# ElesionKyrie/Extreme-Video-Compression-With-Prediction-Using-Pre-trainded-Diffusion-Models-

Hardware: AMD Instinct MI355X
Metric: decoded frames/sec (128x128x30) at q3 (higher is better)
Workload: dtype f32

## Files before the change

### extreme-video-compression-with-prediction-using-pre-trainded-diffusion-models-_amd/csrc/api.hip

```cpp
#include <hip/hip_runtime.h>
#include <string.h>
#include "../../include/evc_hip.h"

extern "C" const char* evc_version(void) { return "evc-hip 0.1"; }
extern "C" const char* evc_arch(void) { return "gfx950"; }

extern "C" int evc_device_ok(void) {
    int dev = 0;
    if (hipGetDevice(&dev) != hipSuccess) return 0;
    hipDeviceProp_t prop;
    if (hipGetDeviceProperties(&prop, dev) != hipSuccess) return 0;
    return strncmp(prop.gcnArchName, "gfx950", 6) == 0 ? 1 : 0;
}

__global__ void clock_probe_kernel(unsigned long long* out, unsigned long long ref_ticks, const unsigned* stop) {
    const unsigned long long r0 = wall_clock64(), c0 = clock64();
    unsigned long long r1 = r0;
    while (r1 - r0 < ref_ticks) {
        __builtin_amdgcn_s_sleep(64);
        r1 = wall_clock64();
        if (stop && __hip_atomic_load(stop, __ATOMIC_RELAXED, __HIP_MEMORY_SCOPE_AGENT) != 0u) break;
    }
    const unsigned long long c1 = clock64();
    if (threadIdx.x == 0) { out[0] = c1 - c0; out[1] = r1 - r0; }
}

extern "C" int evc_clock_probe(unsigned long long* out2, int spin_us, const unsigned* stop, void* stream) {
    if (!out2 || spin_us <= 0 || spin_us > 10000000) return EVC_EINVAL;
    hipLaunchKernelGGL(clock_probe_kernel, dim3(1), dim3(64), 0, (hipStream_t)stream, out2, (unsigned long long)spin_us * 100ull, stop);
    return hipGetLastError() == hipSuccess ? EVC_OK : EVC_ELAUNCH;
}
```

### extreme-video-compression-with-prediction-using-pre-trainded-diffusion-models-_amd/csrc/conv_igemm.hip

```cpp
#include <hip/hip_runtime.h>
#include <stdint.h>
#include <stdio.h>
#include "../../include/evc_hip.h"

typedef float f32x16 __attribute__((ext_vector_type(16)));
typedef __attribute__((address_space(3))) void lds_void;
typedef const __attribute__((address_space(1))) void glb_void;

#ifndef EVC_CONV_TAIL
#define EVC_CONV_TAIL 1
#endif
#ifndef EVC_CONV_TM1
#define EVC_CONV_TM1 1
#endif
#ifndef EVC_SPLIT_WIDE_TILES
#define EVC_SPLIT_WIDE_TILES 1
#endif

#ifndef EVC_SPLIT_INTERLEAVE
#define EVC_SPLIT_INTERLEAVE 5
#endif

namespace {

// ... 1128 lines not shown
        }
    }
}

__device__ __forceinline__ void wide_epilogue(const ConvK& p, f32x16 (&acc)[4][3], char* lds, int m0, int n0, int split,
                                              int wave, int lane, bool tail) {
    const bool partial = p.splits > 1 || tail;
    if (partial) wide_epilogue_t<true, false, false, false>(p, acc, lds, m0, n0, split, wave, lane, tail);
    else if (p.act_out != EVC_ACT_NONE) wide_epilogue_t<false, true, true, true>(p, acc, lds, m0, n0, split, wave, lane, tail);
    else if (p.res && p.stats) wide_epilogue_t<false, true, true, false>(p, acc, lds, m0, n0, split, wave, lane, tail);
    else if (p.stats) wide_epilogue_t<false, false, true, false>(p, acc, lds, m0, n0, split, wave, lane, tail);
    else if (p.res) wide_epilogue_t<false, true, false, false>(p, acc, lds, m0, n0, split, wave, lane, tail);
    else wide_epilogue_t<false, false, false, false>(p, acc, lds, m0, n0, split, wave, lane, tail);
}

#ifndef EVC_WIDE_VMEM_EVERY
#define EVC_WIDE_VMEM_EVERY 36
#endif
#ifndef EVC_WIDE_BDIST
#define EVC_WIDE_BDIST 1
#endif
#ifndef EVC_WIDE_BUFFER_LOADS
#define EVC_WIDE_BUFFER_LOADS 0
#endif
#ifndef EVC_WIDE_ABL
#define EVC_WIDE_ABL 0
#endif
#ifdef EVC_WIDE_STAMPS
__device__ unsigned long long g_wide_stamps[8192 * 8];
#define EVC_STAMP(k) if (threadIdx.x == 0) g_wide_stamps[(blockIdx.x & 8191) * 8 + (k)] = __builtin_readcyclecounter();
#else
#define EVC_STAMP(k)
#endif
template <int MODE, int NU, bool X2>
__global__ __launch_bounds__(256, 1) void conv_wide_kernel(ConvK p) {
    typedef Split<2> SP;
    typedef f16x8 vec;
    constexpr int TM = 4, TN = 3, BM = 256, BN = 192, RB = 32;
    constexpr bool HAS_COEF = MODE == MODE_AFFINE || MODE == MODE_AFFINE_SILU;
    extern __shared__ __attribute__((aligned(16))) char smem_b[];
    const int W = p.W, SW = W + 2;
    const int R = BM / W;
    const int SPX = (R + 2) * SW;
    const int APL = SPX * RB;
    const int HPL = SPX * 16;
    char* const As = smem_b;

    const int tid = threadIdx.x;
    const int lane = tid & 63;
    const int wave = __builtin_amdgcn_readfirstlane(tid >> 6);
    const int wm = wave >> 1, wn = wave & 1;
    const int l31 = lane & 31, half = lane >> 5;

#ifdef EVC_WIDE_STAGGER_TEST
    if (blockIdx.x < 256) for (int q = 0; q < (int)((blockIdx.x >> 3) & 3) * EVC_WIDE_STAGGER_TEST; ++q) __builtin_amdgcn_s_sleep(127);
#endif
    EVC_STAMP(0)
    const bool tail = (int)blockIdx.x >= p.tail_first;
    const int tq = tail ? ((int)blockIdx.x - p.tail_first) / p.tail_splits : 0;
    const int m0 = (tail ? p.tail_first + tq : (int)blockIdx.x) * BM;
    const int n0 = blockIdx.y * BN;
    const int split = tail ? (int)blockIdx.x - p.tail_first - tq * p.tail_splits : (int)blockIdx.z;
    const int sps = tail ? p.tail_sps : p.steps_per_split;
    const int c_begin = p.cut_chunk ? (split ? p.cut_chunk : 0) : min(p.nchunk, split * (sps / 9));
    const int c_end = p.cut_chunk ? (split ? p.nchunk : p.cut_chunk) : min(p.nchunk, c_begin + sps / 9);

    const int bimg = m0 / p.HW;
    const int y0 = (m0 - bimg * p.HW) / W;
// ... 73 lines not shown
            cs[0] = *reinterpret_cast<const float4*>(p.coef_s + co);
            cs[1] = *reinterpret_cast<const float4*>(p.coef_s + co + 4);
        }
    };
    auto stage_store = [&](int k, int buf) {
        vec pl[2];
        SP::split(transform<MODE>(xr[k][0], ca[0], cs[0], sval[k]), transform<MODE>(xr[k][1], ca[1], cs[1], sval[k]), xscale, pl);
        char* A = As + buf * 2 * APL + slds[k];
        *reinterpret_cast<vec*>(A) = pl[0];
        *reinterpret_cast<vec*>(A + APL) = pl[1];
    };
    auto read_a = [&](int i, const char* img, int toff) {
        a[i][0] = *reinterpret_cast<const vec*>(img + abase[i] + toff);
        a[i][1] = *reinterpret_cast<const vec*>(img + APL + abase[i] + toff);
    };

    f32x16 acc[TM][TN];
#pragma unroll
    for (int i = 0; i < TM; ++i)
#pragma unroll
        for (int j = 0; j < TN; ++j)
#pragma unroll
            for (int r = 0; r < 16; ++r) acc[i][j][r] = 0.f;

    vec b[3][TN][2];
    const bool early = !X2 && c_begin < c_end;
    if (early) {
        coef_load(c_begin);
#pragma unroll
        for (int k = 0; k < NU; ++k) stage_load(k, c_begin);
        load_b(b[0], c_begin, 0);
    }
    EVC_STAMP(5)
    {
        const int nimg = X2 ? 3 : 2;
        const int per_img = (R + 2) * 2 * 4;
        for (int u = tid; u < nimg * per_img; u += 256) {
            const int img = u / per_img, q = u - img * per_img;
            const int ph = q & 3, side = (q >> 2) & 1, row = q >> 3;
            const int spx = row * SW + (side ? W + 1 : 0);
            *reinterpret_cast<float4*>(As + img * 2 * APL + (ph >> 1) * APL + (ph & 1) * HPL + spx * 16) = make_float4(0.f, 0.f, 0.f, 0.f);
        }
    }
    __syncthreads();

#define EVC_PIN(x) asm volatile("" : "+v"(x))
#define EVC_PIN4(f) asm volatile("" : "+v"((f).x), "+v"((f).y), "+v"((f).z), "+v"((f).w))
#define EVC_WIDE_MFMA_I(I, BB)                                                                          \
    _Pragma("unroll") for (int t_ = 0; t_ < SP::NTERM; ++t_)                                            \
        _Pragma("unroll") for (int j = 0; j < TN; ++j)                                                  \
            acc[I][j] = SP::mfma(a[I][SP::qa(t_)], BB[j][SP::qb(t_)], acc[I][j]);

    if constexpr (X2) {
        const int nch2 = (p.x2_C0 + p.x2_C1) / KC;
        const int nsp = tail ? p.tail_splits : p.splits;
        const int per = (nch2 + nsp - 1) / nsp;
        const int c2b = min(nch2, split * per), c2e = min(nch2, c2b + per);
        float s2 = 1.0f;
        {
            const float bb = sqrtf(__uint_as_float(p.x2_bound[bound_index(p, m0)]));
            if (!(bb < 3.0e38f)) s2 = __builtin_nanf("");
            else if (bb > 0.f) s2 = ldexpf(1.0f, 6 - ilogbf(bb));
        }
        const float xscale2 = F16_ACT_SCALE * s2;
        const unsigned slab2 = 2u * planeB;
        float4 x2r[2][2][2];
        unsigned x2o0[2], x2o1[2];
        int x2l[2];
#pragma unroll
        for (int k = 0; k < 2; ++k) {
            const int pp = (tid + 256 * k) >> 1;
            const int r = pp / W, x = pp - r * W;
            x2o0[k] = ((unsigned)(m0 + pp) * (unsigned)p.x2_ld0 + 8u * kh) * 4u;
            x2o1[k] = ((unsigned)(m0 + pp) * (unsigned)p.x2_ld1 + 8u * kh) * 4u;
            x2l[k] = kh * HPL + ((r + 1) * SW + x + 1) * 16;
        }
        auto load2 = [&](int c, float4 (&xr2)[2][2]) {
            const int cc = c * KC;
            const bool first = cc < p.x2_C0;
            const char* src = reinterpret_cast<const char*>(first ? p.x2_src0 : p.x2_src1);
            const unsigned cb = (unsigned)(first ? cc : cc - p.x2_C0) * 4u;
#pragma unroll
            for (int k = 0; k < 2; ++k) {
                const unsigned o = (first ? x2o0[k] : x2o1[k]) + cb;
                xr2[k][0] = *reinterpret_cast<const float4*>(src + o);
                xr2[k][1] = *reinterpret_cast<const float4*>(src + o + 16);
            }
        };
        auto store2 = [&](int buf, float4 (&xr2)[2][2]) {
            const float4 z = make_float4(0.f, 0.f, 0.f, 0.f);
#pragma unroll
            for (int k = 0; k < 2; ++k) {
                vec pl[2];
                SP::split(transform<MODE_PLAIN>(xr2[k][0], z, z, true), transform<MODE_PLAIN>(xr2[k][1], z, z, true), xscale2, pl);
                char* A = As + buf * 2 * APL + x2l[k];
                *reinterpret_cast<vec*>(A) = pl[0];
                *reinterpret_cast<vec*>(A + APL) = pl[1];
            }
        };
        vec b2[2][TN][2];
        auto load_b2 = [&](vec (&bb)[TN][2], int c) {
            const char* wt = p.x2_w + (unsigned)c * slab2;
#pragma unroll
            for (int j = 0; j < TN; ++j) {
                bb[j][0] = *reinterpret_cast<const vec*>(wt + wlane + j * 32 * RB);
                bb[j][1] = *reinterpret_cast<const vec*>(wt + planeB + wlane + j * 32 * RB);
            }
        };
        const int n2 = c2e - c2b;
        if (n2 > 0) {
            const auto clampc = [&](int c) { return min(c, c2e - 1); };
            load2(c2b, x2r[0]);
            load2(clampc(c2b + 1), x2r[1]);
            load_b2(b2[0], c2b);
            store2(0, x2r[0]);
            store2(1, x2r[1]);
            load2(clampc(c2b + 2), x2r[0]);
            load2(clampc(c2b + 3), x2r[1]);
            __syncthreads();
#pragma unroll
            for (int i = 0; i < TM; ++i) read_a(i, As, tap_off(4));
            int ring = 0;
#define EVC_WIDE_X2_STEP(BCUR, BNXT, XR)                                                                    \
            {                                                                                           \
                const int rn1 = ring == 2 ? 0 : ring + 1, rn2 = rn1 == 2 ? 0 : rn1 + 1;                 \
                _Pragma("unroll") for (int j = 0; j < TN; ++j) { EVC_PIN(BCUR[j][0]); EVC_PIN(BCUR[j][1]); } \
                _Pragma("unroll") for (int k = 0; k < 2; ++k) { EVC_PIN4(XR[k][0]); EVC_PIN4(XR[k][1]); } \
                load_b2(BNXT, clampc(c + 1));                                                           \
                const char* An = As + rn1 * 2 * APL;                                                    \
                _Pragma("unroll") for (int i = 0; i < TM; ++i) {                                        \
                    EVC_PIN(a[i][0]); EVC_PIN(a[i][1]);                                                 \
                    EVC_WIDE_MFMA_I(i, BCUR)                                                            \
                    read_a(i, An, tap_off(4));                                                          \
                }                                                                                       \
                store2(rn2, XR);                                                       \
                _Pragma("unroll") for (int m = 0; m < 36; ++m) {                                        \
                    if (m == 0) __builtin_amdgcn_sched_group_barrier(0x020, 6, 0);                      \
                    __builtin_amdgcn_sched_group_barrier(0x008, 1, 0);                                  \
                    __builtin_amdgcn_sched_group_barrier(0x402, 3, 0);                                  \
                    if (m % 9 == 8) __builtin_amdgcn_sched_group_barrier(0x100, 2, 0);                  \
                }                                                                                       \
                __builtin_amdgcn_sched_group_barrier(0x200, 4, 0);                                      \
                __builtin_amdgcn_sched_barrier(0);                                                      \
                load2(clampc(c + 4), XR);                                \
                asm volatile("s_waitcnt lgkmcnt(0)\n\ts_barrier" ::: "memory");                         \
                __builtin_amdgcn_sched_barrier(0);                                                      \
                ring = rn1;                                                                             \
            }
            int c = c2b;
            for (; c + 1 < c2e; c += 2) {
                EVC_WIDE_X2_STEP(b2[0], b2[1], x2r[0])
                ++c;
                EVC_WIDE_X2_STEP(b2[1], b2[0], x2r[1])
                --c;
            }
            if (c < c2e) EVC_WIDE_X2_STEP(b2[0], b2[1], x2r[0])
#undef EVC_WIDE_X2_STEP
        }
        __syncthreads();
        const float r = (p.x2_hdr[0] / s2) / (p.w_hdr[0] / in_scale(p, m0));
#pragma unroll
        for (int i = 0; i < TM; ++i)
#pragma unroll
            for (int j = 0; j < TN; ++j)
#pragma unroll
                for (int e = 0; e < 16; ++e) acc[i][j][e] *= r;
    }

    EVC_STAMP(6)
    if (c_begin < c_end) {
        if (!early) {
            coef_load(c_begin);
#pragma unroll
            for (int k = 0; k < NU; ++k) stage_load(k, c_begin);
            load_b(b[0], c_begin, 0);
        }
        if (EVC_WIDE_BDIST == 2) load_b(b[1], c_begin, 1);
#pragma unroll
        for (int k = 0; k < NU; ++k) stage_store(k, 0);
        EVC_STAMP(7)
        __syncthreads();
#pragma unroll
        for (int i = 0; i < TM; ++i) read_a(i, As, 0);
    }
    EVC_STAMP(1)
    for (int c = c_begin; c < c_end; ++c) {
        const int ab = (c - c_begin) & 1;
        const int cn = min(c + 1, c_end - 1);
        const char* Acur = As + ab * 2 * APL;
        const char* Anxt = As + (ab ^ 1) * 2 * APL;
#define EVC_WIDE_STEP(T, LOADK, STOREK, TAIL_CODE)                                                      \
        {                                                                                               \
// ... 30 lines not shown
        EVC_WIDE_STEP(2, 2, 0, )
        EVC_WIDE_STEP(3, 3, 1, )
        EVC_WIDE_STEP(4, -1, 2, )
        EVC_WIDE_STEP(5, -1, 3, )
        EVC_WIDE_STEP(6, -1, -1, )
        EVC_WIDE_STEP(7, -1, -1, asm volatile("s_waitcnt lgkmcnt(0)\n\ts_barrier" ::: "memory");)
        EVC_WIDE_STEP(8, -1, -1, )
#undef EVC_WIDE_STEP
    }
#undef EVC_WIDE_MFMA_I
#undef EVC_PIN
#undef EVC_PIN4

    if (EVC_WIDE_ABL & 16) {
        float sacc = 0.f;
#pragma unroll
        for (int i = 0; i < TM; ++i)
#pragma unroll
            for (int j = 0; j < TN; ++j)
#pragma unroll
                for (int e = 0; e < 16; ++e) sacc += acc[i][j][e];
        p.out[(size_t)m0 * p.ld_out + tid] = sacc;
        return;
    }
    EVC_STAMP(2)
    __syncthreads();
    wide_epilogue(p, acc, As, (EVC_WIDE_ABL & 128) ? 0 : m0, n0, split, wave, lane, tail);
#ifdef EVC_WIDE_STAMPS
    asm volatile("s_waitcnt vmcnt(0)" ::: "memory");
    EVC_STAMP(3)
    if (threadIdx.x == 0) g_wide_stamps[(blockIdx.x & 8191) * 8 + 4] = __builtin_amdgcn_s_getreg(6 | (8 << 6) | (3 << 11)) ;
#endif
}

__global__ __launch_bounds__(1024) void conv_splitk_reduce_kernel(const float* __restrict__ ws, int splits, int M,
                                                                  int Co, const float* __restrict__ bias,
                                                                  const float* __restrict__ res, int ld_res,
                                                                  float scale, int act, float* __restrict__ out,
                                                                  int ld_out, float* __restrict__ stats) {
    __shared__ float red[2][16][64];
    const int l = threadIdx.x & 63;
    const int c = blockIdx.y * 64 + l;
    const int rg = threadIdx.x >> 6;
    const int m_base = blockIdx.x * 64;
    const size_t total = (size_t)M * Co;
    float s_sum = 0.f, s_sq = 0.f;
    if (c < Co) {
        const float b = bias ? bias[c] : 0.f;
        float v[4];
        size_t idx[4];
        bool ok[4];
#pragma unroll
        for (int k = 0; k < 4; ++k) {
            const int m = m_base + rg + 16 * k;
            ok[k] = m < M;
            idx[k] = (size_t)(ok[k] ? m : 0) * Co + c;
            v[k] = 0.f;
        }
        for (int z = 0; z < splits; ++z) {
            const float* w = ws + (size_t)z * total;
#pragma unroll
            for (int k = 0; k < 4; ++k) v[k] += w[idx[k]];
        }
#pragma unroll
        for (int k = 0; k < 4; ++k) {
            if (!ok[k]) continue;
// ... 152 lines not shown
    return hipGetLastError() == hipSuccess ? EVC_OK : EVC_ELAUNCH;
}

static int conv_validate(const evc_conv_args* a) {
    if (!a || !a->src0 || !a->w_packed || !a->out) return EVC_EINVAL;
    if (a->C0 <= 0 || a->C0 % KC != 0 || a->C1 < 0 || a->C1 % KC != 0) return EVC_EINVAL;
    if (a->C1 > 0 && !a->src1) return EVC_EINVAL;
    if ((a->ld0 != 0 && (a->ld0 < a->C0 || (a->ld0 & 3))) || (a->ld1 != 0 && (a->ld1 < a->C1 || (a->ld1 & 3))))
        return EVC_EINVAL;
    if ((a->coef_a == nullptr) != (a->coef_s == nullptr)) return EVC_EINVAL;
    if (a->B <= 0 || a->H <= 0 || a->W <= 0 || a->Co <= 0) return EVC_EINVAL;
    if (a->KH <= 0 || a->KW <= 0 || !(a->KH & 1) || !(a->KW & 1)) return EVC_EINVAL;
    if (a->ld_out < a->Co || (a->res && a->ld_res < a->Co)) return EVC_EINVAL;
    if ((long long)a->B * a->H * a->W > 0x7fffffffLL) return EVC_EINVAL;
    if (a->arith != EVC_ARITH_F32 && a->arith != EVC_ARITH_BF16X6 && a->arith != EVC_ARITH_F16X3) return EVC_EINVAL;
    if (a->x2_w_packed) {
        if (!a->x2_src0 || !a->x2_bound || a->x2_C0 <= 0 || a->x2_C0 % KC != 0 || a->x2_C1 < 0 || a->x2_C1 % KC != 0) return EVC_EINVAL;
        if (a->x2_C1 > 0 && !a->x2_src1) return EVC_EINVAL;
        if ((a->x2_ld0 != 0 && (a->x2_ld0 < a->x2_C0 || (a->x2_ld0 & 3))) || (a->x2_ld1 != 0 && (a->x2_ld1 < a->x2_C1 || (a->x2_ld1 & 3))))
            return EVC_EINVAL;
    }
    return EVC_OK;
}

struct TileCfg { int tm, tn, bm, bn; long long tiles; int splits; int reuse; int wide; int steps_per_split;
                 int tail_first, tail_tiles, tail_splits, tail_sps;
                 int cut_chunk; };
static int g_wide_cut = 1;
static int g_tail_split = EVC_CONV_TAIL;
static int g_wide_tiles = EVC_SPLIT_WIDE_TILES;
static int g_no_reuse = 0;
static int g_wide_mid = 1;
static int g_wide256 = 1;
static int g_force_tm = 0;

static void split_tile_cfg(const evc_conv_args* a, long long M, long long ntile, int nsteps, TileCfg& c, bool rr_ok, bool inv) {
    const double K = (double)a->KH * a->KW * (a->C0 + a->C1);
    const bool f16 = a->arith == EVC_ARITH_F16X3 && rr_ok;
    const double E = f16 ? 20.0 : 6.0, F2 = f16 ? 1.5 : 1.0;
    const auto grid_time = [&](long long n, double sps) {
        const long long R = n / 512, rem = n - R * 512;
        return (sps + E) * ((double)R * F2 + (rem == 0 ? 0.0 : (rem <= 256 && f16 ? 1.0 : F2)));
    };
    double best = 1e300;
    int best_tm = 2, best_s = 1;
    c.tail_first = 0; c.tail_tiles = 0; c.tail_splits = 1; c.tail_sps = 0;
    for (int tm = 2; tm >= 1; --tm) {
        if (!inv && g_force_tm && tm != g_force_tm) continue;
        const long long tiles = ((M + 64 * tm - 1) / (64 * tm)) * ntile;
        const int smax = a->splits > 0 ? a->splits : (nsteps / 4 < 1 ? 1 : (nsteps / 4 > 32 ? 32 : nsteps / 4));
        for (int s = a->splits > 0 ? a->splits : 1; s <= smax; ++s) {
            const double sps = (double)((nsteps + s - 1) / s);
            const double slab_mb = (double)s * (double)M * a->Co * 4.0 / 1e6;
            const double pen = s > 1 ? 1.0 + (slab_mb > 192.0 ? 300.0 : 40.0) * s / K : 1.0;
            const double tmf = tm == 1 ? (a->KH * a->KW > 1 ? 0.5 / (rr_ok ? 0.55 : 0.75) : 0.5) : 1.0;
            const double t = grid_time(tiles * s, sps) * pen * tmf;
            if (t < best * 0.9999) { best = t; best_tm = tm; best_s = s; }
        }
    }
    c.tm = best_tm;
    c.bm = 64 * c.tm;
    c.tiles = ((M + c.bm - 1) / c.bm) * ntile;
    c.splits = best_s;
    if (!inv && rr_ok && g_tail_split && a->splits <= 0 && !g_force_tm && M % 128 == 0) {
        const long long tm_all = M / 128, wgs = tm_all * ntile;
        const long long R = wgs / 512;
        const long long main_m = R * 512 / ntile, tail_m = tm_all - main_m;
        const int unit = 3 * 9;
        if (R >= 1 && tail_m > 0 && nsteps >= 2 * unit) {
            int ts = (int)(512 / (tail_m * ntile));
            if (ts > nsteps / unit) ts = nsteps / unit;
            if (ts >= 2) {
                int sps = (nsteps + ts - 1) / ts;
                sps = (sps + 2) / 3 * 3;
                ts = (nsteps + sps - 1) / sps;
                const double t_tail = grid_time(main_m * ntile, (double)nsteps) +
                                      grid_time(tail_m * ntile * ts, (double)sps) * (1.0 + 40.0 * ts / K);
                if (ts >= 2 && t_tail < best * 0.98) {
                    c.tm = 2; c.bm = 128; c.tiles = wgs; c.splits = 1;
                    c.tail_first = (int)main_m; c.tail_tiles = (int)tail_m; c.tail_splits = ts; c.tail_sps = sps;
                }
            }
        }
    }
}

static inline bool is_split_arith(int arith) { return arith == EVC_ARITH_BF16X6 || arith == EVC_ARITH_F16X3; }
static inline int arith_planes(int arith) { return arith == EVC_ARITH_F16X3 ? 2 : 3; }
constexpr long long LDS_CAP = 160 * 1024;

static long long rr_lds_bytes(int np, int bm, int W, int bn) {
    return (long long)np * 32 * (2LL * (bm / W) * (W + 2) + 2LL * bn);
}

static long long wide_lds_bytes(int W, bool x2) { return (x2 ? 6LL : 4LL) * (256 / W + 2) * (W + 2) * 32; }

static bool wide_ok(const evc_conv_args* a, bool inv) {
    const bool mode_ok = a->coef_a ? a->act_in == EVC_ACT_SILU : a->act_in == EVC_ACT_NONE;
    return (inv || g_wide256) && mode_ok && a->arith == EVC_ARITH_F16X3 && a->KH == 3 && a->KW == 3 && a->Co % 192 == 0 &&
           (a->W == 16 || a->W == 32 || a->W == 64 || a->W == 128) && ((long long)a->H * a->W) % 256 == 0 &&
           a->ld_out % 4 == 0 && (!a->res || a->ld_res % 4 == 0);
}

static TileCfg conv_tile_cfg_at(const evc_conv_args* a, bool inv) {
    TileCfg c;
    c.wide = 0;
    c.cut_chunk = 0;
    const long long M = (long long)a->B * a->H * a->W;
    const int CoPad = evc_conv_co_pad(a->Co);
    c.tn = pick_tn(CoPad);
    c.bn = 64 * c.tn;
    const long long ntile = CoPad / c.bn;
    const int nsteps = a->KH * a->KW * ((a->C0 + a->C1) / KC);
    c.reuse = 0;
    if (is_split_arith(a->arith)) {
        const int np = arith_planes(a->arith);
        const bool rr_ok = (inv || !g_no_reuse) && a->KH == 3 && a->KW == 3 && a->W >= 4 && 128 % a->W == 0 &&
                           rr_lds_bytes(np, 128, a->W, c.bn) <= LDS_CAP;
        split_tile_cfg(a, M, ntile, nsteps, c, rr_ok, inv);
        if (rr_ok && c.tm == 2) c.reuse = 1;
        if (!inv && c.reuse && c.splits == 1 && !c.tail_tiles && g_wide_tiles && M % 256 == 0 && rr_lds_bytes(np, 256, a->W, c.bn) <= LDS_CAP) {
            const long long t256 = (M / 256) * ntile;
            if ((t256 >= 512 && t256 % 256 == 0) || t256 >= 6 * 256) {
                c.bm = 256;
                c.tiles = t256;
            }
        }
    } else {
        c.tail_first = 0; c.tail_tiles = 0; c.tail_splits = 1; c.tail_sps = 0;
        c.tm = (!EVC_CONV_TM1 || ((M + 127) / 128) * ntile >= 64) ? 2 : 1;
        if (g_force_tm && !inv) c.tm = g_force_tm;
        c.bm = 64 * c.tm;
        c.tiles = ((M + c.bm - 1) / c.bm) * ntile;
        long long splits = 1;
        if (a->splits > 0) splits = a->splits;
        else if (c.tiles < 384) {
            splits = (640 + c.tiles / 2) / c.tiles;
            const int max_by_steps = nsteps / 8 > 0 ? nsteps / 8 : 1;
            if (splits > max_by_steps) splits = max_by_steps;
            if (splits > 32) splits = 32;
            if (splits < 1) splits = 1;
        }
        c.splits = (int)splits;
    }
    if (wide_ok(a, inv) && a->splits <= 0 && (inv || !g_force_tm)) {
        const long long tm_all = M / 256, nt = a->Co / 192, wgs = tm_all * nt;
        if (wgs >= 256) {
            const int nchunk = (a->C0 + a->C1) / KC;
            c.wide = 1; c.reuse = 0; c.tm = 4; c.tn = 3; c.bm = 256; c.bn = 192; c.tiles = wgs; c.splits = 1;
            c.tail_first = 0; c.tail_tiles = 0; c.tail_splits = 1; c.tail_sps = 0;
            const long long Rr = wgs / 256;
            const long long main_m = Rr * 256 / nt, tail_m = tm_all - main_m;
            if (!inv && g_tail_split && tail_m > 0) {
                int ts = (int)(256 / (tail_m * nt));
                if (ts > nchunk / 3) ts = nchunk / 3;
                if (ts >= 2) {
                    const int cps = (nchunk + ts - 1) / ts;
                    ts = (nchunk + cps - 1) / cps;
                    c.tail_first = (int)main_m; c.tail_tiles = (int)tail_m; c.tail_splits = ts; c.tail_sps = cps * 9;
                }
            }
            c.steps_per_split = nsteps;
            return c;
        }
        if ((inv || g_wide_mid) && wgs >= 32) {
            const int nchunk = (a->C0 + a->C1) / KC;
            int best_s = 0;
            double best_t = 1e300;
            for (int sp = 1; sp <= 8 && wgs * sp <= 256 && nchunk / sp >= 4; ++sp) {
                const int cps = (nchunk + sp - 1) / sp;
                const double slab_mb = sp > 1 ? (double)sp * M * a->Co * 4.0 / 1e6 : 0.0;
                const double t = 23000.0 + 13900.0 * cps + (sp > 1 ? 2.0 * 2000.0 * (5.0 + slab_mb / 4.0) : 0.0);
                if (t < best_t) { best_t = t; best_s = sp; }
            }
            if (best_s > 0 && wgs * best_s >= 128) {
                const int cps = (nchunk + best_s - 1) / best_s;
                c.wide = 1; c.reuse = 0; c.tm = 4; c.tn = 3; c.bm = 256; c.bn = 192; c.tiles = wgs;
// ... 17 lines not shown
            }
        }
    }
    const int unit = c.reuse ? a->KW : 1;
    int sps = (nsteps + c.splits - 1) / c.splits;
    sps = (sps + unit - 1) / unit * unit;
    c.steps_per_split = sps;
    c.splits = (nsteps + sps - 1) / sps;
    return c;
}

#define EVC_INVARIANT_PLAN_REVISION 1
static TileCfg conv_tile_cfg(const evc_conv_args* a) {
    if (!a->invariant) return conv_tile_cfg_at(a, false);
    evc_conv_args r = *a;
    r.B = EVC_INVARIANT_REF_BATCH;
    TileCfg c = conv_tile_cfg_at(&r, true);
    const long long M = (long long)a->B * a->H * a->W;
    c.tiles = ((M + c.bm - 1) / c.bm) * (evc_conv_co_pad(a->Co) / c.bn);
    return c;
}

extern "C" int evc_invariant_plan_revision(void) { return EVC_INVARIANT_PLAN_REVISION; }

extern "C" int evc_conv_set_option(const char* name, int value) {
    if (!name) return EVC_EINVAL;
    const auto is = [&](const char* s) { int i = 0; while (s[i] && s[i] == name[i]) ++i; return s[i] == 0 && name[i] == 0; };
    if (is("wide_tiles")) { g_wide_tiles = value; return EVC_OK; }
    if (is("row_reuse")) { g_no_reuse = !value; return EVC_OK; }
    if (is("tail_split")) { g_tail_split = value; return EVC_OK; }
    if (is("wide256")) { g_wide256 = value; return EVC_OK; }
    if (is("wide_mid")) { g_wide_mid = value; return EVC_OK; }
    if (is("wide_cut")) { g_wide_cut = value; return EVC_OK; }
    return EVC_EINVAL;
}

extern "C" int evc_conv_fused_1x1_supported(const evc_conv_args* a) {
    if (conv_validate(a) != EVC_OK) return 0;
    if (a->arith != EVC_ARITH_F16X3 || a->KH != 3 || a->KW != 3) return 0;
    const TileCfg c = conv_tile_cfg(a);
    if (a->invariant && ((long long)a->H * a->W) % c.bm != 0) return 0;
    return (c.reuse == 1 || c.wide) ? 1 : 0;
}

extern "C" int evc_conv_kernel_name(const evc_conv_args* a, char* buf, int n) {
    if (!buf || n <= 0 || conv_validate(a) != EVC_OK) return EVC_EINVAL;
    int mode;
    if (a->coef_a) mode = a->act_in == EVC_ACT_SILU ? MODE_AFFINE_SILU : MODE_AFFINE;
    else mode = a->act_in == EVC_ACT_SILU ? MODE_SILU : a->act_in == EVC_ACT_RELU ? MODE_RELU : MODE_PLAIN;
    const TileCfg c = conv_tile_cfg(a);
    int len;
    if (c.wide) len = snprintf(buf, n, "conv_wide_kernel<%d, %d, %s>", mode, a->W == 128 ? 4 : 3, a->x2_w_packed ? "true" : "false");
    else if (is_split_arith(a->arith)) {
        const int np = arith_planes(a->arith);
        if (c.reuse) len = snprintf(buf, n, "conv_split_rr_kernel<%d, %d, %d, %d>", np, c.bm == 256 ? 4 : 2, c.tn, mode);
        else if (np == 3) len = snprintf(buf, n, "conv_split_kernel<%d, %d, %d>", c.tm, c.tn, mode);
        else len = snprintf(buf, n, "conv_splitn_kernel<2, %d, %d, %d>", c.tm, c.tn, mode);
    } else len = snprintf(buf, n, "conv_igemm_kernel<%d, %d, %d>", c.tm, c.tn, mode);
    return len;
}

extern "C" int evc_conv_choose_splits(const evc_conv_args* a) {
    if (conv_validate(a) != EVC_OK) return EVC_EINVAL;
    return conv_tile_cfg(a).splits;
}

extern "C" int evc_conv_stats_splits(const evc_conv_args* a) {
    if (conv_validate(a) != EVC_OK) return 0;
    const int HW = a->H * a->W;
    if (HW % 64 != 0) return 0;
    const TileCfg c = conv_tile_cfg(a);
    if (c.splits > 1 || c.wide) return HW / 64;
    if (a->invariant && HW % c.bm != 0) return 0;
    const long long M = (long long)a->B * HW;
    const int CoPad = evc_conv_co_pad(a->Co);
    if (M % c.bm != 0 || a->Co != CoPad || a->Co % c.bn != 0) return 0;
    return HW / (32 * c.tm);
}

extern "C" int evc_conv_plan_query(const evc_conv_args* a, evc_conv_plan* out) {
    if (!out || conv_validate(a) != EVC_OK) return EVC_EINVAL;
    const TileCfg c = conv_tile_cfg(a);
    if (evc_conv_kernel_name(a, out->kernel, (int)sizeof(out->kernel)) < 0) return EVC_EINVAL;
    out->tile_m = c.bm; out->tile_n = c.bn; out->splits = c.splits; out->steps_per_split = c.steps_per_split;
    out->cut_chunk = c.wide ? c.cut_chunk : 0;
// ... 55 lines not shown
template <int TM, int TN>
static int launch_split2(int mode, dim3 grid, size_t lds, hipStream_t st, const ConvK& k) {
#define EVC_CALL(M) hipLaunchKernelGGL((conv_splitn_kernel<2, TM, TN, M>), grid, dim3(256), lds, st, k)
    EVC_MODE_SWITCH(mode, EVC_CALL)
#undef EVC_CALL
    return EVC_OK;
}

template <int NP, int WM, int TN, int MODE>
static int launch_split_rr_one(dim3 grid, size_t lds, hipStream_t st, const ConvK& k) {
    static unsigned long long attr_done = 0;
    const int rc = ensure_dynamic_lds(reinterpret_cast<const void*>(&conv_split_rr_kernel<NP, WM, TN, MODE>), &attr_done, lds);
    if (rc != EVC_OK) return rc;
    hipLaunchKernelGGL((conv_split_rr_kernel<NP, WM, TN, MODE>), grid, dim3(128 * WM), lds, st, k);
    return EVC_OK;
}
template <int NP, int WM, int TN>
static int launch_split_rr(int mode, dim3 grid, size_t lds, hipStream_t st, const ConvK& k) {
    int rc = EVC_OK;
#define EVC_CALL(M) rc = launch_split_rr_one<NP, WM, TN, M>(grid, lds, st, k)
    EVC_MODE_SWITCH(mode, EVC_CALL)
#undef EVC_CALL
    return rc;
}

template <int MODE, int NU, bool X2>
static int launch_wide_one(dim3 grid, size_t lds, hipStream_t st, const ConvK& k) {
    static unsigned long long attr_done = 0;
    const int rc = ensure_dynamic_lds(reinterpret_cast<const void*>(&conv_wide_kernel<MODE, NU, X2>), &attr_done, lds);
    if (rc != EVC_OK) return rc;
    hipLaunchKernelGGL((conv_wide_kernel<MODE, NU, X2>), grid, dim3(256), lds, st, k);
    return EVC_OK;
}
template <int MODE>
static int launch_wide_mode(int nu, bool x2, dim3 grid, size_t lds, hipStream_t st, const ConvK& k) {
    if (nu == 4) return x2 ? launch_wide_one<MODE, 4, true>(grid, lds, st, k) : launch_wide_one<MODE, 4, false>(grid, lds, st, k);
    return x2 ? launch_wide_one<MODE, 3, true>(grid, lds, st, k) : launch_wide_one<MODE, 3, false>(grid, lds, st, k);
}
static int launch_wide(int mode, int nu, bool x2, dim3 grid, size_t lds, hipStream_t st, const ConvK& k) {
#ifdef EVC_DEV_FAST
    return launch_wide_mode<MODE_AFFINE_SILU>(nu, x2, grid, lds, st, k);
#else
    if (mode == MODE_AFFINE_SILU) return launch_wide_mode<MODE_AFFINE_SILU>(nu, x2, grid, lds, st, k);
    if (mode == MODE_PLAIN) return launch_wide_mode<MODE_PLAIN>(nu, x2, grid, lds, st, k);
    return EVC_EUNSUPPORTED;
#endif
}

#define EVC_TN_SWITCH(tn, CALL) ((tn) == 3 ? CALL(3) : (tn) == 2 ? CALL(2) : CALL(1))

static int conv2d_impl(const evc_conv_args* a, float* ws, void* stream, hipEvent_t ev_start, hipEvent_t ev_conv_end);

extern "C" int evc_conv2d_nhwc_f32(const evc_conv_args* a, float* ws, void* stream) {
    return conv2d_impl(a, ws, stream, nullptr, nullptr);
}

extern "C" int evc_conv2d_nhwc_profiled_f32(const evc_conv_args* a, float* ws, void* stream, void* ev_start,
                                            void* ev_conv_end) {
    return conv2d_impl(a, ws, stream, (hipEvent_t)ev_start, (hipEvent_t)ev_conv_end);
}

static int conv2d_impl(const evc_conv_args* a, float* ws, void* stream, hipEvent_t ev_start, hipEvent_t ev_conv_end) {
    int rc = conv_validate(a);
    if (rc != EVC_OK) return rc;
    int mode;
    if (a->coef_a) {
        if (a->act_in == EVC_ACT_SILU) mode = MODE_AFFINE_SILU;
        else if (a->act_in == EVC_ACT_NONE) mode = MODE_AFFINE;
        else return EVC_EUNSUPPORTED;
    } else {
        mode = a->act_in == EVC_ACT_SILU ? MODE_SILU : a->act_in == EVC_ACT_RELU ? MODE_RELU : MODE_PLAIN;
        if (a->act_in != EVC_ACT_NONE && a->act_in != EVC_ACT_SILU && a->act_in != EVC_ACT_RELU) return EVC_EINVAL;
    }
    ConvK k;
    k.src0 = a->src0; k.src1 = a->src1 ? a->src1 : a->src0; k.C0 = a->C0; k.C1 = a->C1;
    k.ld0 = a->ld0 > 0 ? a->ld0 : a->C0; k.ld1 = a->ld1 > 0 ? a->ld1 : (a->C1 > 0 ? a->C1 : k.ld0);
    k.coef_a = a->coef_a; k.coef_s = a->coef_s;
// ... 25 lines not shown
    if (a->stats_out && evc_conv_stats_splits(a) == 0) return EVC_EINVAL;
    k.x2_w = nullptr; k.x2_hdr = nullptr; k.x2_bound = nullptr; k.x2_src0 = k.x2_src1 = nullptr;
    k.x2_C0 = k.x2_C1 = k.x2_ld0 = k.x2_ld1 = 0;
    if (a->x2_w_packed) {
        if (a->arith != EVC_ARITH_F16X3 || a->KH != 3 || a->KW != 3 || !(cfg.reuse == 1 || cfg.wide)) return EVC_EUNSUPPORTED;
        k.x2_src0 = a->x2_src0; k.x2_src1 = a->x2_src1 ? a->x2_src1 : a->x2_src0;
        k.x2_C0 = a->x2_C0; k.x2_C1 = a->x2_C1;
        k.x2_ld0 = a->x2_ld0 > 0 ? a->x2_ld0 : a->x2_C0;
        k.x2_ld1 = a->x2_ld1 > 0 ? a->x2_ld1 : (a->x2_C1 > 0 ? a->x2_C1 : k.x2_ld0);
        if ((long long)k.M * k.x2_ld0 * 4 >= (1LL << 32) || (long long)k.M * k.x2_ld1 * 4 >= (1LL << 32)) return EVC_EUNSUPPORTED;
        k.x2_hdr = a->x2_w_packed;
        k.x2_w = reinterpret_cast<const char*>(a->x2_w_packed) + F16_HDR_BYTES;
        k.x2_bound = a->x2_bound;
    }
    k.bound_stride = 0; k.generic_epi = 0;
    if (a->invariant) {
        const bool whole = k.HW % cfg.bm == 0;
        k.bound_stride = 1;
        k.generic_epi = whole ? 0 : 1;
        if (!whole && (cfg.reuse || cfg.wide) && (a->in_bound || a->x2_w_packed)) return EVC_EUNSUPPORTED;
    }
    k.tail_first = 0x7fffffff; k.tail_splits = 1; k.tail_sps = 0; k.tail_rows = 0;
    k.cut_chunk = cfg.wide ? cfg.cut_chunk : 0;
    if (cfg.tail_tiles) {
        k.tail_first = cfg.tail_first; k.tail_splits = cfg.tail_splits; k.tail_sps = cfg.tail_sps;
        k.tail_rows = cfg.tail_tiles * cfg.bm;
    }

    dim3 grid((k.M + cfg.bm - 1) / cfg.bm, k.CoPad / cfg.bn, k.splits);
    if (cfg.tail_tiles) grid.x = cfg.tail_first + cfg.tail_tiles * cfg.tail_splits;
    hipStream_t st = (hipStream_t)stream;
    if (ev_start && hipEventRecord(ev_start, st) != hipSuccess) return EVC_ELAUNCH;
    if (cfg.wide) {
        rc = launch_wide(mode, a->W == 128 ? 4 : 3, a->x2_w_packed != nullptr, grid, (size_t)wide_lds_bytes(a->W, a->x2_w_packed != nullptr), st, k);
    } else if (is_split_arith(a->arith)) {
        const int np = arith_planes(a->arith);
        if (cfg.reuse) {
            const size_t lds_rr = (size_t)rr_lds_bytes(np, cfg.bm, a->W, cfg.bn);
#define EVC_RR4_3(TN) launch_split_rr<3, 4, TN>(mode, grid, lds_rr, st, k)
#define EVC_RR2_3(TN) launch_split_rr<3, 2, TN>(mode, grid, lds_rr, st, k)
#define EVC_RR4_2(TN) launch_split_rr<2, 4, TN>(mode, grid, lds_rr, st, k)
#define EVC_RR2_2(TN) launch_split_rr<2, 2, TN>(mode, grid, lds_rr, st, k)
            if (np == 3) rc = cfg.bm == 256 ? EVC_TN_SWITCH(cfg.tn, EVC_RR4_3) : EVC_TN_SWITCH(cfg.tn, EVC_RR2_3);
            else rc = cfg.bm == 256 ? EVC_TN_SWITCH(cfg.tn, EVC_RR4_2) : EVC_TN_SWITCH(cfg.tn, EVC_RR2_2);
#undef EVC_RR4_3
#undef EVC_RR2_3
#undef EVC_RR4_2
#undef EVC_RR2_2
        } else {
            const size_t lds = (size_t)2 * np * (cfg.bm + cfg.bn) * 32;
#define EVC_S3_2(TN) launch_split3<2, TN>(mode, grid, lds, st, k)
#define EVC_S3_1(TN) launch_split3<1, TN>(mode, grid, lds, st, k)
#define EVC_S2_2(TN) launch_split2<2, TN>(mode, grid, lds, st, k)
#define EVC_S2_1(TN) launch_split2<1, TN>(mode, grid, lds, st, k)
            if (np == 3) rc = cfg.tm == 2 ? EVC_TN_SWITCH(cfg.tn, EVC_S3_2) : EVC_TN_SWITCH(cfg.tn, EVC_S3_1);
            else rc = cfg.tm == 2 ? EVC_TN_SWITCH(cfg.tn, EVC_S2_2) : EVC_TN_SWITCH(cfg.tn, EVC_S2_1);
#undef EVC_S3_2
#undef EVC_S3_1
#undef EVC_S2_2
#undef EVC_S2_1
        }
    } else {
        const size_t lds = (size_t)2 * (cfg.bm + cfg.bn) * KC * sizeof(float);
#define EVC_F_2(TN) launch_mode<2, TN>(mode, grid, lds, st, k)
#define EVC_F_1(TN) launch_mode<1, TN>(mode, grid, lds, st, k)
        rc = cfg.tm == 2 ? EVC_TN_SWITCH(cfg.tn, EVC_F_2) : EVC_TN_SWITCH(cfg.tn, EVC_F_1);
#undef EVC_F_2
// ... 22 lines not shown
```

Before: 38.11.

## Add grouped multi-buffered LDS ring for fused 1x1 phase of wide conv

Adds a grouped variant of the wide conv kernel in which the fused 1x1 (x2) operand phase uses a ring of 2*G unpadded LDS buffers and synchronises only once per group of G chunks, instead of after every chunk. The halo-zeroing pass moves after that phase so its barrier is no longer needed up front. The grouped kernel with G=4 becomes the default for non-invariant calls. The cost is a larger LDS footprint and more complex hand scheduling with explicit s_barrier, plus the risk of race bugs in the ring indexing.

```diff
diff --git a/extreme-video-compression-with-prediction-using-pre-trainded-diffusion-models-_amd/csrc/api.hip b/extreme-video-compression-with-prediction-using-pre-trainded-diffusion-models-_amd/csrc/api.hip
--- a/extreme-video-compression-with-prediction-using-pre-trainded-diffusion-models-_amd/csrc/api.hip
+++ b/extreme-video-compression-with-prediction-using-pre-trainded-diffusion-models-_amd/csrc/api.hip
@@ -4,6 +4,8 @@
 
 extern "C" const char* evc_version(void) { return "evc-hip 0.1"; }
 extern "C" const char* evc_arch(void) { return "gfx950"; }
+
+extern "C" const int evc_wide_x2_group_default = 4;
 
 extern "C" int evc_device_ok(void) {
     int dev = 0;
diff --git a/extreme-video-compression-with-prediction-using-pre-trainded-diffusion-models-_amd/csrc/conv_igemm.hip b/extreme-video-compression-with-prediction-using-pre-trainded-diffusion-models-_amd/csrc/conv_igemm.hip
--- a/extreme-video-compression-with-prediction-using-pre-trainded-diffusion-models-_amd/csrc/conv_igemm.hip
+++ b/extreme-video-compression-with-prediction-using-pre-trainded-diffusion-models-_amd/csrc/conv_igemm.hip
@@ -1184,8 +1184,9 @@
 #else
 #define EVC_STAMP(k)
 #endif
-template <int MODE, int NU, bool X2>
-__global__ __launch_bounds__(256, 1) void conv_wide_kernel(ConvK p) {
+template <int MODE, int NU, bool X2, int G>
+__device__ __forceinline__ void conv_wide_body(ConvK p) {
+    static_assert(G == 1 || (X2 && (G == 2 || G == 4)), "grouped 1x1 phase: G = 2 or 4, fused operand only");
     typedef Split<2> SP;
     typedef f16x8 vec;
     constexpr int TM = 4, TN = 3, BM = 256, BN = 192, RB = 32;
@@ -1325,7 +1326,7 @@
         load_b(b[0], c_begin, 0);
     }
     EVC_STAMP(5)
-    {
+    if constexpr (G == 1) {
         const int nimg = X2 ? 3 : 2;
         const int per_img = (R + 2) * 2 * 4;
         for (int u = tid; u < nimg * per_img; u += 256) {
@@ -1334,8 +1335,8 @@
             const int spx = row * SW + (side ? W + 1 : 0);
             *reinterpret_cast<float4*>(As + img * 2 * APL + (ph >> 1) * APL + (ph & 1) * HPL + spx * 16) = make_float4(0.f, 0.f, 0.f, 0.f);
         }
-    }
-    __syncthreads();
+        __syncthreads();
+    }
 
 #define EVC_PIN(x) asm volatile("" : "+v"(x))
 #define EVC_PIN4(f) asm volatile("" : "+v"((f).x), "+v"((f).y), "+v"((f).z), "+v"((f).w))
@@ -1357,6 +1358,8 @@
         }
         const float xscale2 = F16_ACT_SCALE * s2;
         const unsigned slab2 = 2u * planeB;
+        constexpr int HPL2 = BM * 16 + 64, APL2 = 2 * HPL2, IMG2 = 2 * APL2;
+        const int img_b = G == 1 ? 2 * APL : IMG2, pl_b = G == 1 ? APL : APL2;
         float4 x2r[2][2][2];
         unsigned x2o0[2], x2o1[2];
         int x2l[2];
@@ -1366,7 +1369,7 @@
             const int r = pp / W, x = pp - r * W;
             x2o0[k] = ((unsigned)(m0 + pp) * (unsigned)p.x2_ld0 + 8u * kh) * 4u;
             x2o1[k] = ((unsigned)(m0 + pp) * (unsigned)p.x2_ld1 + 8u * kh) * 4u;
-            x2l[k] = kh * HPL + ((r + 1) * SW + x + 1) * 16;
+            x2l[k] = G == 1 ? kh * HPL + ((r + 1) * SW + x + 1) * 16 : kh * HPL2 + pp * 16;
         }
         auto load2 = [&](int c, float4 (&xr2)[2][2]) {
             const int cc = c * KC;
@@ -1386,9 +1389,9 @@
             for (int k = 0; k < 2; ++k) {
                 vec pl[2];
                 SP::split(transform<MODE_PLAIN>(xr2[k][0], z, z, true), transform<MODE_PLAIN>(xr2[k][1], z, z, true), xscale2, pl);
-                char* A = As + buf * 2 * APL + x2l[k];
+                char* A = As + buf * img_b + x2l[k];
                 *reinterpret_cast<vec*>(A) = pl[0];
-                *reinterpret_cast<vec*>(A + APL) = pl[1];
+                *reinterpret_cast<vec*>(A + pl_b) = pl[1];
             }
         };
         vec b2[2][TN][2];
@@ -1401,7 +1404,7 @@
             }
         };
         const int n2 = c2e - c2b;
-        if (n2 > 0) {
+        if (G == 1 && n2 > 0) {
             const auto clampc = [&](int c) { return min(c, c2e - 1); };
             load2(c2b, x2r[0]);
             load2(clampc(c2b + 1), x2r[1]);
@@ -1450,7 +1453,82 @@
             if (c < c2e) EVC_WIDE_X2_STEP(b2[0], b2[1], x2r[0])
 #undef EVC_WIDE_X2_STEP
         }
+        if (G > 1 && n2 > 0) {
+            const auto clampc = [&](int c) { return min(c, c2e - 1); };
+            const int abase2 = half * HPL2 + (wm * 128 + l31) * 16;
+            const auto read_a2 = [&](int i, const char* img) {
+                a[i][0] = *reinterpret_cast<const vec*>(img + abase2 + i * 512);
+                a[i][1] = *reinterpret_cast<const vec*>(img + APL2 + abase2 + i * 512);
+            };
+            {
+                float4 xp[G + 1][2][2];
+                load2(c2b, xp[0]);
+#pragma unroll
+                for (int j = 1; j <= G; ++j)
+                    if (j < n2) load2(c2b + j, xp[j]);
+                load_b2(b2[0], c2b);
+                store2(0, xp[0]);
+#pragma unroll
+                for (int j = 1; j <= G; ++j)
+                    if (j < n2) store2(j, xp[j]);
+            }
+            load2(clampc(c2b + G + 1), x2r[0]);
+            load2(clampc(c2b + G + 2), x2r[1]);
+            __syncthreads();
+#pragma unroll
+            for (int i = 0; i < TM; ++i) read_a2(i, As);
+            int gb = 0;
+#define EVC_WIDE_X2G_STEP(K)                                                                                \
+            {                                                                                           \
+                auto& bcur = b2[(K) & 1];                                                               \
+                auto& bnxt = b2[((K) + 1) & 1];                                                         \
+                auto& xr2 = x2r[(K) & 1];                                                               \
+                int rs = gb + (K) + 1, ws = gb + (K) + 1 + G;                                           \
+                if (rs >= 2 * G) rs -= 2 * G;                                                           \
+                if (ws >= 2 * G) ws -= 2 * G;                                                           \
+                _Pragma("unroll") for (int j = 0; j < TN; ++j) { EVC_PIN(bcur[j][0]); EVC_PIN(bcur[j][1]); } \
+                _Pragma("unroll") for (int k = 0; k < 2; ++k) { EVC_PIN4(xr2[k][0]); EVC_PIN4(xr2[k][1]); } \
+                load_b2(bnxt, clampc(c + (K) + 1));                                                     \
+                const char* An = As + rs * IMG2;                                                        \
+                _Pragma("unroll") for (int i = 0; i < TM; ++i) {                                        \
+                    EVC_PIN(a[i][0]); EVC_PIN(a[i][1]);                                                 \
+                    EVC_WIDE_MFMA_I(i, bcur)                                                            \
+                    read_a2(i, An);                                                                     \
+                }                                                                                       \
+                store2(ws, xr2);                                               \
+                _Pragma("unroll") for (int m = 0; m < 36; ++m) {                                        \
+                    if (m == 0) __builtin_amdgcn_sched_group_barrier(0x020, 6, 0);                      \
+                    __builtin_amdgcn_sched_group_barrier(0x008, 1, 0);                                  \
+                    __builtin_amdgcn_sched_group_barrier(0x402, 3, 0);                                  \
+                    if (m % 9 == 8) __builtin_amdgcn_sched_group_barrier(0x100, 2, 0);                  \
+                }                                                                                       \
+                __builtin_amdgcn_sched_group_barrier(0x200, 4, 0);                                      \
+                __builtin_amdgcn_sched_barrier(0);                                                      \
+                load2(clampc(c + (K) + G + 3), xr2);                     \
+                if ((K) == G - 2) asm volatile("s_waitcnt lgkmcnt(0)\n\ts_barrier" ::: "memory");       \
+                __builtin_amdgcn_sched_barrier(0);                                                      \
+            }
+            for (int c = c2b; c < c2e; c += G) {
+                EVC_WIDE_X2G_STEP(0)
+                if (c + 1 < c2e) EVC_WIDE_X2G_STEP(1)
+                if constexpr (G > 2) {
+                    if (c + 2 < c2e) EVC_WIDE_X2G_STEP(2)
+                    if (c + 3 < c2e) EVC_WIDE_X2G_STEP(3)
+                }
+                gb = G - gb;
+            }
+#undef EVC_WIDE_X2G_STEP
+        }
         __syncthreads();
+        if constexpr (G > 1) {
+            const int per_img = (R + 2) * 2 * 4;
+            for (int u = tid; u < 2 * per_img; u += 256) {
+                const int img = u / per_img, q = u - img * per_img;
+                const int ph = q & 3, side = (q >> 2) & 1, row = q >> 3;
+                const int spx = row * SW + (side ? W + 1 : 0);
+                *reinterpret_cast<float4*>(As + img * 2 * APL + (ph >> 1) * APL + (ph & 1) * HPL + spx * 16) = make_float4(0.f, 0.f, 0.f, 0.f);
+            }
+        }
         const float r = (p.x2_hdr[0] / s2) / (p.w_hdr[0] / in_scale(p, m0));
 #pragma unroll
         for (int i = 0; i < TM; ++i)
@@ -1547,6 +1625,10 @@
     if (threadIdx.x == 0) g_wide_stamps[(blockIdx.x & 8191) * 8 + 4] = __builtin_amdgcn_s_getreg(6 | (8 << 6) | (3 << 11)) ;
 #endif
 }
+template <int MODE, int NU, bool X2>
+__global__ __launch_bounds__(256, 1) void conv_wide_kernel(ConvK p) { conv_wide_body<MODE, NU, X2, 1>(p); }
+template <int MODE, int NU, int G>
+__global__ __launch_bounds__(256, 1) void conv_wide_kernel_x2g(ConvK p) { conv_wide_body<MODE, NU, true, G>(p); }
 
 __global__ __launch_bounds__(1024) void conv_splitk_reduce_kernel(const float* __restrict__ ws, int splits, int M,
                                                                   int Co, const float* __restrict__ bias,
@@ -1765,6 +1847,9 @@
 static int g_no_reuse = 0;
 static int g_wide_mid = 1;
 static int g_wide256 = 1;
+extern "C" const int evc_wide_x2_group_default;
+static int g_wide_x2_group = 0;
+static int g_wide_force = 0;
 static int g_force_tm = 0;
 
 static void split_tile_cfg(const evc_conv_args* a, long long M, long long ntile, int nsteps, TileCfg& c, bool rr_ok, bool inv) {
@@ -1826,7 +1911,17 @@
     return (long long)np * 32 * (2LL * (bm / W) * (W + 2) + 2LL * bn);
 }
 
-static long long wide_lds_bytes(int W, bool x2) { return (x2 ? 6LL : 4LL) * (256 / W + 2) * (W + 2) * 32; }
+static long long wide_lds_bytes(int W, bool x2, int x2g) {
+    const long long img = 2LL * (256 / W + 2) * (W + 2) * 32;
+    if (!x2 || x2g <= 1) return (x2 ? 3LL : 2LL) * img;
+    const long long ring = 2LL * x2g * 4 * (256 * 16 + 64);
+    return ((ring > 2 * img ? ring : 2 * img) + 2559) / 2560 * 2560;
+}
+static_assert(2LL * 4 * 4 * (256 * 16 + 64) <= LDS_CAP, "ring of the grouped 1x1 phase");
+static int wide_x2_group(const evc_conv_args* a) {
+    const int g = a->invariant ? 0 : g_wide_x2_group;
+    return g ? g : (evc_wide_x2_group_default == 2 || evc_wide_x2_group_default == 4 ? evc_wide_x2_group_default : 1);
+}
 
 static bool wide_ok(const evc_conv_args* a, bool inv) {
     const bool mode_ok = a->coef_a ? a->act_in == EVC_ACT_SILU : a->act_in == EVC_ACT_NONE;
@@ -1876,6 +1971,14 @@
         }
         c.splits = (int)splits;
     }
+    if (!inv && g_wide_force && !g_force_tm && wide_ok(a, inv)) {
+        const int nchunk = (a->C0 + a->C1) / KC, s = a->splits > 0 ? a->splits : 1;
+        c.wide = 1; c.reuse = 0; c.tm = 4; c.tn = 3; c.bm = 256; c.bn = 192; c.tiles = (M / 256) * (a->Co / 192);
+        c.tail_first = 0; c.tail_tiles = 0; c.tail_splits = 1; c.tail_sps = 0;
+        c.splits = s;
+        c.steps_per_split = (nchunk + s - 1) / s * 9;
+        return c;
+    }
     if (wide_ok(a, inv) && a->splits <= 0 && (inv || !g_force_tm)) {
         const long long tm_all = M / 256, nt = a->Co / 192, wgs = tm_all * nt;
         if (wgs >= 256) {
@@ -1959,6 +2062,12 @@
     if (is("wide256")) { g_wide256 = value; return EVC_OK; }
     if (is("wide_mid")) { g_wide_mid = value; return EVC_OK; }
     if (is("wide_cut")) { g_wide_cut = value; return EVC_OK; }
+    if (is("wide_force")) { g_wide_force = value; return EVC_OK; }
+    if (is("wide_x2_group")) {
+        if (value != 0 && value != 1 && value != 2 && value != 4) return EVC_EINVAL;
+        g_wide_x2_group = value;
+        return EVC_OK;
+    }
     return EVC_EINVAL;
 }
 
@@ -1977,7 +2086,9 @@
     else mode = a->act_in == EVC_ACT_SILU ? MODE_SILU : a->act_in == EVC_ACT_RELU ? MODE_RELU : MODE_PLAIN;
     const TileCfg c = conv_tile_cfg(a);
     int len;
-    if (c.wide) len = snprintf(buf, n, "conv_wide_kernel<%d, %d, %s>", mode, a->W == 128 ? 4 : 3, a->x2_w_packed ? "true" : "false");
+    if (c.wide && a->x2_w_packed && wide_x2_group(a) > 1)
+        len = snprintf(buf, n, "conv_wide_kernel_x2g<%d, %d, %d>", mode, a->W == 128 ? 4 : 3, wide_x2_group(a));
+    else if (c.wide) len = snprintf(buf, n, "conv_wide_kernel<%d, %d, %s>", mode, a->W == 128 ? 4 : 3, a->x2_w_packed ? "true" : "false");
     else if (is_split_arith(a->arith)) {
         const int np = arith_planes(a->arith);
         if (c.reuse) len = snprintf(buf, n, "conv_split_rr_kernel<%d, %d, %d, %d>", np, c.bm == 256 ? 4 : 2, c.tn, mode);
@@ -2099,17 +2210,27 @@
     hipLaunchKernelGGL((conv_wide_kernel<MODE, NU, X2>), grid, dim3(256), lds, st, k);
     return EVC_OK;
 }
+template <int MODE, int NU, int G>
+static int launch_wide_x2g_one(dim3 grid, size_t lds, hipStream_t st, const ConvK& k) {
+    static unsigned long long attr_done = 0;
+    const int rc = ensure_dynamic_lds(reinterpret_cast<const void*>(&conv_wide_kernel_x2g<MODE, NU, G>), &attr_done, lds);
+    if (rc != EVC_OK) return rc;
+    hipLaunchKernelGGL((conv_wide_kernel_x2g<MODE, NU, G>), grid, dim3(256), lds, st, k);
+    return EVC_OK;
+}
 template <int MODE>
-static int launch_wide_mode(int nu, bool x2, dim3 grid, size_t lds, hipStream_t st, const ConvK& k) {
+static int launch_wide_mode(int nu, bool x2, int x2g, dim3 grid, size_t lds, hipStream_t st, const ConvK& k) {
+    if (x2 && x2g == 4) return nu == 4 ? launch_wide_x2g_one<MODE, 4, 4>(grid, lds, st, k) : launch_wide_x2g_one<MODE, 3, 4>(grid, lds, st, k);
+    if (x2 && x2g == 2) return nu == 4 ? launch_wide_x2g_one<MODE, 4, 2>(grid, lds, st, k) : launch_wide_x2g_one<MODE, 3, 2>(grid, lds, st, k);
     if (nu == 4) return x2 ? launch_wide_one<MODE, 4, true>(grid, lds, st, k) : launch_wide_one<MODE, 4, false>(grid, lds, st, k);
     return x2 ? launch_wide_one<MODE, 3, true>(grid, lds, st, k) : launch_wide_one<MODE, 3, false>(grid, lds, st, k);
 }
-static int launch_wide(int mode, int nu, bool x2, dim3 grid, size_t lds, hipStream_t st, const ConvK& k) {
+static int launch_wide(int mode, int nu, bool x2, int x2g, dim3 grid, size_t lds, hipStream_t st, const ConvK& k) {
 #ifdef EVC_DEV_FAST
-    return launch_wide_mode<MODE_AFFINE_SILU>(nu, x2, grid, lds, st, k);
+    return launch_wide_mode<MODE_AFFINE_SILU>(nu, x2, x2g, grid, lds, st, k);
 #else
-    if (mode == MODE_AFFINE_SILU) return launch_wide_mode<MODE_AFFINE_SILU>(nu, x2, grid, lds, st, k);
-    if (mode == MODE_PLAIN) return launch_wide_mode<MODE_PLAIN>(nu, x2, grid, lds, st, k);
+    if (mode == MODE_AFFINE_SILU) return launch_wide_mode<MODE_AFFINE_SILU>(nu, x2, x2g, grid, lds, st, k);
+    if (mode == MODE_PLAIN) return launch_wide_mode<MODE_PLAIN>(nu, x2, x2g, grid, lds, st, k);
     return EVC_EUNSUPPORTED;
 #endif
 }
@@ -2201,7 +2322,9 @@
     hipStream_t st = (hipStream_t)stream;
     if (ev_start && hipEventRecord(ev_start, st) != hipSuccess) return EVC_ELAUNCH;
     if (cfg.wide) {
-        rc = launch_wide(mode, a->W == 128 ? 4 : 3, a->x2_w_packed != nullptr, grid, (size_t)wide_lds_bytes(a->W, a->x2_w_packed != nullptr), st, k);
+        const bool x2 = a->x2_w_packed != nullptr;
+        const int x2g = x2 ? wide_x2_group(a) : 1;
+        rc = launch_wide(mode, a->W == 128 ? 4 : 3, x2, x2g, grid, (size_t)wide_lds_bytes(a->W, x2, x2g), st, k);
     } else if (is_split_arith(a->arith)) {
         const int np = arith_planes(a->arith);
         if (cfg.reuse) {
```

New measurement: 38.25, median of 6. No clear change (+0.4%).
